# natir/br

Measured on AMD Instinct MI355X. Metric: corrected Gbases/sec at k=19, 10 kb ONT-error reads, higher is better.
Workload: dtype u64 k-mers / 1-bit set

## Files before the change

### br_amd/csrc/brx_partbuild.hip

```cpp
#include "brx_internal.hpp"
#include "brx_index.hpp"

#include <stdlib.h>
#include <string.h>
#include <atomic>

using namespace brx;

namespace {

constexpr int F_BITS = 12;
constexpr int MAX_LEVELS = 4;
constexpr int MAX_DIGIT_BITS = 9;
static_assert(MAX_DIGIT_BITS <= 9, "the digit scans of the partition passes are written for at most 512 digits");

struct Plan {
    int k, nbits, nlev;
    int bits[MAX_LEVELS];
    int rem_in[MAX_LEVELS];
    uint64_t nchild[MAX_LEVELS];
};

Plan make_plan(int k)
{
    Plan p;
    memset(&p, 0, sizeof(p));
    p.k = k;
    p.nbits = 2 * k - 1;
    const int P = p.nbits - F_BITS;
    p.nlev = (P + MAX_DIGIT_BITS - 1) / MAX_DIGIT_BITS;
    if (p.nlev < 2)
        p.nlev = 2;
    int left = P, rem = p.nbits;
    uint64_t nb = 1;
    for (int l = 0; l < p.nlev; l++) {
        int b = (left + (p.nlev - l) - 1) / (p.nlev - l);
        if (l == 0 && p.nbits - b > 32)
            b = p.nbits - 32;
        p.bits[l] = b;
        p.rem_in[l] = rem;
        rem -= b;
        left -= b;
        nb <<= b;
        p.nchild[l] = nb;
    }
    return p;
}

__device__ __forceinline__ uint32_t pack4(uint32_t w)
{
    uint32_t x = __builtin_bswap32((w >> 1) & 0x03030303u);
    x |= x >> 6;
    return (x | (x >> 12)) & 0xffu;
}

#ifndef BRX_L1_UNROLL
#define BRX_L1_UNROLL 4
#endif
#ifndef BRX_XCD_ITEMS
#define BRX_XCD_ITEMS 1
#endif
#ifndef BRX_DEBUG_BOUNDS
#define BRX_DEBUG_BOUNDS 0
#endif
#if BRX_DEBUG_BOUNDS
__device__ unsigned long long bounds_violations = 0ull;
__device__ __forceinline__ bool store_ok(uint64_t idx, uint64_t cap)
{
    if (idx >= cap) {
        atomicAdd(&bounds_violations, 1ull);
        return false;
    }
    return true;
}
#else
__device__ __forceinline__ bool store_ok(uint64_t, uint64_t) { return true; }
#endif
constexpr bool XCD_ITEMS = BRX_XCD_ITEMS != 0;
constexpr uint32_t L1_TILE = 4096;
constexpr uint32_t PACK_WORDS = L1_TILE / 16 + 4;
constexpr uint32_t BND_WORDS = (L1_TILE + 64) / 32 + 2;

__device__ __forceinline__ void pack_window(const uint8_t *__restrict__ bases, uint64_t total, uint64_t g0, uint32_t nbases,
                                            uint32_t *__restrict__ pk)
{
    const uint32_t nwords = (nbases + 15u) / 16u;
    for (uint32_t w = threadIdx.x; w < nwords; w += 256) {
        const uint64_t p = g0 + 16ull * w;
        uint32_t v[4] = {0, 0, 0, 0};
        if (p + 16 <= total) {
            uint4 q;
            __builtin_memcpy(&q, bases + p, 16);
            v[0] = q.x; v[1] = q.y; v[2] = q.z; v[3] = q.w;
        } else {
            for (uint32_t j = 0; j < 16; j++)
                if (p + j < total)
                    v[j >> 2] |= (uint32_t)bases[p + j] << (8u * (j & 3u));
        }
        pk[w] = (pack4(v[0]) << 24) | (pack4(v[1]) << 16) | (pack4(v[2]) << 8) | pack4(v[3]);
    }
}

__device__ __forceinline__ uint64_t kmer_at(const uint32_t *__restrict__ pk, uint32_t pos, int k)
{
    const uint32_t w = pos >> 4, sh = 2u * (pos & 15u);
    const uint64_t hi = ((uint64_t)pk[w] << 32) | pk[w + 1];
    const uint64_t lo = pk[w + 2];
    const uint64_t val = sh ? ((hi << sh) | (lo >> (32u - sh))) : hi;
    return val >> (64 - 2 * k);
}

struct ItemRange {
    unsigned long long first, end, step;
};
__device__ __forceinline__ ItemRange xcd_items(unsigned long long n_items)
{
    const unsigned long long G = gridDim.x, b = blockIdx.x;
    if (G < 8ull || !XCD_ITEMS)
        return {b, n_items, G};
    const unsigned long long x = b & 7ull, j = b >> 3;
    const unsigned long long R = (n_items + 7ull) >> 3;
    const unsigned long long lo = x * R;
    unsigned long long hi = lo + R;
    if (hi > n_items)
        hi = n_items;
    return {lo + j, hi, (G - x + 7ull) >> 3};
}

struct L1Args {
    const uint8_t *bases;
    const uint64_t *offsets;
    uint32_t n_reads;
    uint64_t total;
    uint32_t n_items;
    int k, nbits, bits;
    uint32_t *matrix;
    uint32_t n_ranges;
    uint64_t *rsum;
    const uint64_t *coff;
    uint32_t *keys_out;
    uint64_t out_cap;
};

__device__ __forceinline__ void l1_prepare(const L1Args &a, uint32_t item, uint32_t *pk, uint32_t *bnd, uint32_t *sh_r0,
                                           uint32_t &n_here, bool search)
{
    const uint64_t off0 = a.offsets[0];
    const uint64_t g0 = (uint64_t)item * L1_TILE;
    const uint64_t left = a.total - g0;
    n_here = (uint32_t)(left < L1_TILE ? left : L1_TILE);
    const uint32_t win = n_here + (uint32_t)a.k + 32u;
    pack_window(a.bases + off0, a.total, g0, win, pk);
    for (uint32_t w = threadIdx.x; w < BND_WORDS; w += 256)
        bnd[w] = 0;
    if (threadIdx.x == 0) {
        if (search) {
            uint32_t lo = 0, hi = a.n_reads + 1;
            while (lo < hi) {
                const uint32_t mid = lo + (hi - lo) / 2;
                if (a.offsets[mid] - off0 <= g0)
                    lo = mid + 1;
                else
                    hi = mid;
            }
            sh_r0[0] = lo;
        } else {
            sh_r0[0] += sh_r0[1];
        }
        sh_r0[1] = 0;
    }
    __syncthreads();
    const uint64_t lim = g0 + n_here + (uint64_t)a.k;
    uint32_t before_next = 0;
    for (uint32_t r = sh_r0[0] + threadIdx.x; r <= a.n_reads; r += 256) {
        const uint64_t o = a.offsets[r] - off0;
        if (o >= lim)
            break;
        const uint32_t p = (uint32_t)(o - g0);
        atomicOr(&bnd[p >> 5], 1u << (p & 31u));
        before_next += o <= g0 + L1_TILE ? 1u : 0u;
    }
    if (before_next)
        atomicAdd(&sh_r0[1], before_next);
    __syncthreads();
}

__device__ __forceinline__ void l1_range(uint32_t n_items, uint32_t &lo, uint32_t &hi)
{
    lo = (uint32_t)(((uint64_t)blockIdx.x * n_items) / gridDim.x);
    hi = (uint32_t)(((uint64_t)(blockIdx.x + 1) * n_items) / gridDim.x);
}

struct L1Next {
    uint4 q0, q1;
    uint64_t off;
    uint32_t m[(1u << MAX_DIGIT_BITS) / 256u];
};

__device__ __forceinline__ uint32_t l1_window_words(const L1Args &a, uint32_t item, uint32_t &n_here)
{
    const uint64_t left = a.total - (uint64_t)item * L1_TILE;
    n_here = (uint32_t)(left < L1_TILE ? left : L1_TILE);
    return (n_here + (uint32_t)a.k + 32u + 15u) / 16u;
}

template <bool ROW>
__device__ __forceinline__ void l1_fetch(const L1Args &a, uint64_t off0, uint32_t item, uint32_t r_first, L1Next &nx)
{
    const uint8_t *bases = a.bases + off0;
    const uint64_t g0 = (uint64_t)item * L1_TILE;
    uint32_t n_here;
    const uint32_t nwords = l1_window_words(a, item, n_here);
    const uint64_t p0 = g0 + 16ull * threadIdx.x, p1 = p0 + 16ull * 256ull;
    nx.q0 = make_uint4(0, 0, 0, 0);
    nx.q1 = make_uint4(0, 0, 0, 0);
    if (threadIdx.x < nwords && p0 + 16 <= a.total)
        __builtin_memcpy(&nx.q0, bases + p0, 16);
    if (256u + threadIdx.x < nwords && p1 + 16 <= a.total)
        __builtin_memcpy(&nx.q1, bases + p1, 16);
    const uint32_t r = r_first + threadIdx.x;
    nx.off = a.offsets[r <= a.n_reads ? r : a.n_reads];
    if (ROW) {
        const uint32_t B = 1u << a.bits;
#pragma unroll
        for (uint32_t q = 0; q < (1u << MAX_DIGIT_BITS) / 256u; q++) {
            const uint32_t b = threadIdx.x + 256u * q;
            nx.m[q] = b < B ? a.matrix[(uint64_t)item * B + b] : 0u;
        }
    }
}

template <bool ROW>
__device__ __forceinline__ void l1_landed(const L1Next &nx)
{
    asm volatile("" ::"v"(nx.q0.x), "v"(nx.q0.y), "v"(nx.q0.z), "v"(nx.q0.w), "v"(nx.q1.x), "v"(nx.q1.y), "v"(nx.q1.z), "v"(nx.q1.w),
                 "v"(nx.off));
    if (ROW) {
#pragma unroll
        for (uint32_t q = 0; q < (1u << MAX_DIGIT_BITS) / 256u; q++)
            asm volatile("" ::"v"(nx.m[q]));
    }
}

__device__ __forceinline__ uint32_t l1_pack16(const L1Args &a, uint64_t off0, const uint4 &q, uint64_t p)
{
    uint32_t v[4] = {q.x, q.y, q.z, q.w};
    if (p + 16 > a.total) {
        const uint8_t *bases = a.bases + off0;
        v[0] = v[1] = v[2] = v[3] = 0;
        for (uint32_t j = 0; j < 16; j++)
            if (p + j < a.total)
                v[j >> 2] |= (uint32_t)bases[p + j] << (8u * (j & 3u));
    }
    return (pack4(v[0]) << 24) | (pack4(v[1]) << 16) | (pack4(v[2]) << 8) | pack4(v[3]);
}

__device__ __forceinline__ void l1_consume(const L1Args &a, uint64_t off0, uint32_t item, const L1Next &nx, uint32_t r_first, uint32_t *pk,
                                           uint32_t *bnd, uint32_t *sh_r0, uint32_t &n_here)
{
    const uint64_t g0 = (uint64_t)item * L1_TILE;
    const uint32_t nwords = l1_window_words(a, item, n_here);
    if (threadIdx.x < nwords)
        pk[threadIdx.x] = l1_pack16(a, off0, nx.q0, g0 + 16ull * threadIdx.x);
    if (256u + threadIdx.x < nwords)
        pk[256u + threadIdx.x] = l1_pack16(a, off0, nx.q1, g0 + 16ull * (256u + threadIdx.x));
    for (uint32_t w = threadIdx.x; w < BND_WORDS; w += 256)
        bnd[w] = 0;
    const uint64_t lim = g0 + n_here + (uint64_t)a.k;
    const uint32_t r = r_first + threadIdx.x;
    const uint64_t o = nx.off - off0;
    const bool mine = r <= a.n_reads && o < lim;
    if (threadIdx.x == 0)
        sh_r0[1] = 0;
    if (threadIdx.x == 255)
        sh_r0[2] = mine ? 1u : 0u;
    __syncthreads();
    if (mine) {
        uint32_t p = (uint32_t)(o - g0);
        atomicOr(&bnd[p >> 5], 1u << (p & 31u));
        uint32_t before_next = o <= g0 + L1_TILE ? 1u : 0u;
        if (sh_r0[2])
            for (uint32_t r2 = r + 256u; r2 <= a.n_reads; r2 += 256u) {
                const uint64_t o2 = a.offsets[r2] - off0;
                if (o2 >= lim)
                    break;
                p = (uint32_t)(o2 - g0);
                atomicOr(&bnd[p >> 5], 1u << (p & 31u));
                before_next += o2 <= g0 + L1_TILE ? 1u : 0u;
            }
        if (before_next)
            atomicAdd(&sh_r0[1], before_next);
    }
}

__device__ __forceinline__ void l1_search(const L1Args &a, uint64_t off0, uint32_t item, uint32_t *sh_r0)
{
    if (threadIdx.x == 0) {
        const uint64_t g0 = (uint64_t)item * L1_TILE;
        uint32_t lo = 0, hi = a.n_reads + 1;
        while (lo < hi) {
            const uint32_t mid = lo + (hi - lo) / 2;
            if (a.offsets[mid] - off0 <= g0)
                lo = mid + 1;
            else
                hi = mid;
        }
        sh_r0[0] = lo;
    }
    __syncthreads();
}

__device__ __forceinline__ bool l1_valid(const uint32_t *bnd, uint32_t p, int k)
{
    const uint32_t q = p + 1u;
    const uint32_t w = q >> 5, sh = q & 31u;
    const uint64_t two = ((uint64_t)bnd[w + 1] << 32) | bnd[w];
    const uint32_t bits = (uint32_t)(two >> sh) & ((k > 1) ? ((1u << (k - 1)) - 1u) : 0u);
    return bits == 0u;
}

static_assert(L1_TILE == 256u * 16u, "l1_for_each_hash: 16 positions per thread");
template <int UNROLL = 4, typename F>
__device__ __forceinline__ void l1_for_each_hash(const uint32_t *__restrict__ pk, const uint32_t *__restrict__ bnd, uint32_t n_here,
                                                 int k, F &&f)
{
    const uint32_t p0 = threadIdx.x * 16u;
    if (p0 >= n_here)
        return;
    const uint32_t w = threadIdx.x;
    const uint64_t hi = ((uint64_t)pk[w] << 32) | pk[w + 1];
    const uint64_t lo = pk[w + 2];
    const uint64_t mask = kmask(k);
    uint64_t fwd = hi >> (64 - 2 * k);
    uint64_t rc = revcomp(fwd, k);
    uint64_t next = (hi << (2 * k)) | (2 * k >= 32 ? lo << (2 * k - 32) : lo >> (32 - 2 * k));
    const uint32_t q = p0 + 1u, wq = q >> 5, sh = q & 31u;
    uint64_t vb = ((((uint64_t)bnd[wq + 1] << 32) | bnd[wq]) >> sh) | (sh ? (uint64_t)bnd[wq + 2] << (64u - sh) : 0ull);
    const uint64_t vmask = k > 1 ? (1ull << (k - 1)) - 1ull : 0ull;
    const uint32_t left = n_here - p0 < 16u ? n_here - p0 : 16u;
    const int top = 2 * k - 2;
#pragma unroll UNROLL
    for (uint32_t j = 0; j < left; j++) {
        if ((vb & vmask) == 0ull)
            f(((popc64(fwd) & 1) ? rc : fwd) >> 1);
        const uint64_t b = next >> 62;
        next <<= 2;
        vb >>= 1;
        fwd = ((fwd << 2) | b) & mask;
        rc = (rc >> 2) | ((b ^ 2ull) << top);
    }
}

#ifndef BRX_L1HIST_WAVES
#define BRX_L1HIST_WAVES 1
#endif
constexpr uint32_t L1_OWN = ((1u << MAX_DIGIT_BITS) + 255u) / 256u;

__global__ __launch_bounds__(256, BRX_L1HIST_WAVES) void l1_hist_kernel(L1Args a)
{
    extern __shared__ uint32_t lds[];
    __shared__ uint32_t pk[PACK_WORDS];
    __shared__ uint32_t bnd[BND_WORDS];
    __shared__ uint32_t sh_r0[3];
    const uint32_t B = 1u << a.bits;
    const int shift = a.nbits - a.bits;
    uint32_t lo, hi;
    l1_range(a.n_items, lo, hi);
    uint64_t rs[L1_OWN];
#pragma unroll
    for (uint32_t q = 0; q < L1_OWN; q++)
        rs[q] = 0;
    if (lo < hi) {
        const uint64_t off0 = a.offsets[0];
        l1_search(a, off0, lo, sh_r0);
        uint32_t r_first = sh_r0[0];
        L1Next nx;
        l1_fetch<false>(a, off0, lo, r_first, nx);
        for (uint32_t b = threadIdx.x; b < B; b += 256)
            lds[b] = 0;
        uint32_t n_here;
        l1_landed<false>(nx);
        l1_consume(a, off0, lo, nx, r_first, pk, bnd, sh_r0, n_here);
        __syncthreads();
        r_first += sh_r0[1];
        l1_fetch<false>(a, off0, lo + 1 < hi ? lo + 1 : lo, r_first, nx);
        for (uint32_t item = lo; item < hi; item++) {
            l1_for_each_hash(pk, bnd, n_here, a.k, [&](uint64_t h) { atomicAdd(&lds[(uint32_t)(h >> shift)], 1u); });
            __syncthreads();
            uint32_t row[L1_OWN];
#pragma unroll
            for (uint32_t q = 0; q < L1_OWN; q++) {
                const uint32_t b = threadIdx.x + 256u * q;
                row[q] = 0;
                if (b < B) {
                    row[q] = lds[b];
                    lds[b] = 0;
                }
            }
            l1_landed<false>(nx);
            if (item + 1 < hi) {
                l1_consume(a, off0, item + 1, nx, r_first, pk, bnd, sh_r0, n_here);
                __syncthreads();
                r_first += sh_r0[1];
            }
#pragma unroll
            for (uint32_t q = 0; q < L1_OWN; q++) {
                const uint32_t b = threadIdx.x + 256u * q;
                if (b < B)
                    a.matrix[(uint64_t)item * B + b] = row[q];
                rs[q] += row[q];
            }
            l1_fetch<false>(a, off0, item + 2 < hi ? item + 2 : hi - 1, r_first, nx);
        }
    }
#pragma unroll
    for (uint32_t q = 0; q < L1_OWN; q++) {
        const uint32_t b = threadIdx.x + 256u * q;
        if (b < B && store_ok((uint64_t)blockIdx.x * B + b, (uint64_t)a.n_ranges * B))
            a.rsum[(uint64_t)blockIdx.x * B + b] = rs[q];
    }
}

__global__ __launch_bounds__(256) void col_scan_columns_kernel(uint64_t *__restrict__ part, uint32_t n_rows, uint32_t B,
                                                               uint64_t *__restrict__ coltot)
{
    __shared__ uint64_t wsum[4];
    const uint32_t b = blockIdx.x;
    const uint32_t per = (n_rows + 255u) / 256u;
    const uint32_t c0 = threadIdx.x * per;
    uint64_t mine = 0;
    for (uint32_t q = 0; q < per; q++) {
        const uint32_t c = c0 + q;
        if (c < n_rows)
            mine += part[(uint64_t)c * B + b];
    }
    uint64_t incl = mine;
    for (int d = 1; d < 64; d <<= 1) {
        const uint64_t t = __shfl_up(incl, d);
        if ((threadIdx.x & 63) >= (unsigned)d)
            incl += t;
    }
    if ((threadIdx.x & 63) == 63)
        wsum[threadIdx.x >> 6] = incl;
    __syncthreads();
    uint64_t base = 0;
    for (uint32_t w = 0; w < (threadIdx.x >> 6); w++)
        base += wsum[w];
    uint64_t run = base + incl - mine;
    for (uint32_t q = 0; q < per; q++) {
        const uint32_t c = c0 + q;
        if (c < n_rows) {
            const uint64_t v = part[(uint64_t)c * B + b];
            part[(uint64_t)c * B + b] = run;
            run += v;
        }
    }
    if (threadIdx.x == 255)
        coltot[b] = base + incl;
}

__global__ __launch_bounds__(64) void col_scan_digits_kernel(const uint64_t *__restrict__ coltot, uint32_t B, uint64_t *__restrict__ coff,
                                                             unsigned long long *__restrict__ total)
{
    uint64_t carry = 0;
    for (uint32_t b0 = 0; b0 < B; b0 += 64) {
        const uint32_t b = b0 + threadIdx.x;
        const uint64_t v = b < B ? coltot[b] : 0;
        uint64_t incl = v;
        for (int d = 1; d < 64; d <<= 1) {
            const uint64_t t = __shfl_up(incl, d);
            if (threadIdx.x >= (unsigned)d)
                incl += t;
        }
        if (b < B)
            coff[b] = carry + incl - v;
        carry += __shfl(incl, 63);
    }
    if (threadIdx.x == 0) {
        coff[B] = carry;
        *total = carry;
    }
}

template <bool TABLE>
__global__ __launch_bounds__(256) void flat_insert_kernel(L1Args a, uint32_t *__restrict__ bits, uint64_t *__restrict__ lines,
                                                          uint32_t line_shift, uint32_t m, uint32_t w,
                                                          unsigned long long *__restrict__ n_new)
{
    __shared__ uint32_t pk[PACK_WORDS];
    __shared__ uint32_t bnd[BND_WORDS];
    __shared__ uint32_t sh_r0[2];
    uint32_t added = 0;
    uint32_t lo, hi;
    l1_range(a.n_items, lo, hi);
    for (uint32_t item = lo; item < hi; item++) {
        uint32_t n_here;
        l1_prepare(a, item, pk, bnd, sh_r0, n_here, item == lo);
        for (uint32_t p = threadIdx.x; p < n_here; p += 256)
            if (l1_valid(bnd, p, a.k)) {
                const uint64_t kmer = kmer_at(pk, p, a.k);
                if (TABLE) {
                    added += table_find_or_insert(lines, line_shift, m, w, a.k, kmer) ? 1u : 0u;
                } else {
                    const uint64_t h = khash(kmer, a.k);
                    atomicOr(bits + (h >> 5), 1u << (h & 31u));
                }
            }
        __syncthreads();
    }
    if (TABLE) {
        for (int d = 32; d > 0; d >>= 1)
            added += __shfl_down(added, d);
        if ((threadIdx.x & 63) == 0 && added)
            atomicAdd(n_new, (unsigned long long)added);
    }
}

__global__ __launch_bounds__(256) void flat_count_kernel(L1Args a, uint64_t *__restrict__ lines, uint32_t *__restrict__ counts,
                                                         uint32_t line_shift, uint32_t m, uint32_t w, unsigned long long *__restrict__ n_new)
{
    __shared__ uint32_t pk[PACK_WORDS];
    __shared__ uint32_t bnd[BND_WORDS];
    __shared__ uint32_t sh_r0[2];
    uint32_t added = 0;
    uint32_t lo, hi;
    l1_range(a.n_items, lo, hi);
    for (uint32_t item = lo; item < hi; item++) {
        uint32_t n_here;
        l1_prepare(a, item, pk, bnd, sh_r0, n_here, item == lo);
        for (uint32_t p = threadIdx.x; p < n_here; p += 256)
            if (l1_valid(bnd, p, a.k)) {
                bool fresh;
                const uint64_t slot = table_find_or_claim(lines, line_shift, m, w, a.k, kmer_at(pk, p, a.k), fresh);
                added += fresh ? 1u : 0u;
                table_count_bump(counts + slot);
            }
        __syncthreads();
    }
    for (int d = 32; d > 0; d >>= 1)
        added += __shfl_down(added, d);
// ... 11 lines not shown
    seen++;
    kmer = kmer_at(pk, p, a.k);
    return table_owner_of(khash(kmer, a.k), parts) == part;
}

__global__ __launch_bounds__(256) void flat_count_slice_kernel(L1Args a, uint64_t *__restrict__ lines, uint32_t *__restrict__ counts,
                                                               uint32_t line_shift, uint32_t m, uint32_t w, uint32_t part, uint32_t parts,
                                                               unsigned long long *__restrict__ n_new,
                                                               unsigned long long *__restrict__ stats4)
{
    __shared__ uint32_t pk[PACK_WORDS];
    __shared__ uint32_t bnd[BND_WORDS];
    __shared__ uint32_t sh_r0[2];
    __shared__ uint64_t queue[4][SLICE_QUEUE];
    uint64_t *q = queue[threadIdx.x >> 6];
    const uint32_t lane = threadIdx.x & 63u;
    const unsigned long long below = (1ull << lane) - 1ull;
    uint32_t added = 0, seen = 0;
    uint32_t head = 0, queued = 0, trips = 0;
    unsigned long long walked = 0;
    uint32_t lo, hi;
    l1_range(a.n_items, lo, hi);
    for (uint32_t item = lo; item < hi; item++) {
        uint32_t n_here;
        l1_prepare(a, item, pk, bnd, sh_r0, n_here, item == lo);
        for (uint32_t p0 = 0; p0 < n_here; p0 += 256) {
            uint64_t kmer = 0;
            const bool mine = slice_take(a, pk, bnd, p0 + threadIdx.x, n_here, part, parts, kmer, seen);
            const unsigned long long mask = __ballot(mine);
            if (mine)
                q[(head + queued + (uint32_t)__popcll(mask & below)) & (SLICE_QUEUE - 1u)] = kmer;
            queued += (uint32_t)__popcll(mask);
            if (queued >= 64u) {
                __builtin_amdgcn_wave_barrier();
                const uint64_t mer = q[(head + lane) & (SLICE_QUEUE - 1u)];
                __builtin_amdgcn_wave_barrier();
                head = (head + 64u) & (SLICE_QUEUE - 1u);
                queued -= 64u;
                bool fresh;
                const uint64_t slot = table_find_or_claim(lines, line_shift, m, w, a.k, mer, fresh);
                added += fresh ? 1u : 0u;
                table_count_bump(counts + slot);
                walked += 64ull;
                trips++;
            }
        }
        __syncthreads();
    }
    if (queued) {
        __builtin_amdgcn_wave_barrier();
        if (lane < queued) {
            bool fresh;
            const uint64_t slot = table_find_or_claim(lines, line_shift, m, w, a.k, q[(head + lane) & (SLICE_QUEUE - 1u)], fresh);
            added += fresh ? 1u : 0u;
            table_count_bump(counts + slot);
        }
        walked += queued;
        trips++;
    }
    for (int d = 32; d > 0; d >>= 1) {
        added += __shfl_down(added, d);
        seen += __shfl_down(seen, d);
    }
    if (lane == 0u) {
        if (added)
            atomicAdd(n_new, (unsigned long long)added);
        if (seen)
            atomicAdd(stats4 + 0, (unsigned long long)seen);
        if (walked)
            atomicAdd(stats4 + 1, walked);
        if (trips)
            atomicAdd(stats4 + 2, (unsigned long long)trips);
        atomicAdd(stats4 + 3, 1ull);
    }
}

__global__ __launch_bounds__(256) void flat_slice_census_kernel(L1Args a, uint32_t part, uint32_t parts, unsigned long long *__restrict__ out2)
{
    __shared__ uint32_t pk[PACK_WORDS];
    __shared__ uint32_t bnd[BND_WORDS];
    __shared__ uint32_t sh_r0[2];
    uint32_t owned = 0, seen = 0;
    uint32_t lo, hi;
    l1_range(a.n_items, lo, hi);
    for (uint32_t item = lo; item < hi; item++) {
        uint32_t n_here;
        l1_prepare(a, item, pk, bnd, sh_r0, n_here, item == lo);
        for (uint32_t p = threadIdx.x; p < n_here; p += 256) {
            uint64_t kmer;
            owned += slice_take(a, pk, bnd, p, n_here, part, parts, kmer, seen) ? 1u : 0u;
        }
        __syncthreads();
    }
    for (int d = 32; d > 0; d >>= 1) {
        owned += __shfl_down(owned, d);
        seen += __shfl_down(seen, d);
    }
    if ((threadIdx.x & 63) == 0 && seen) {
        atomicAdd(out2 + 0, (unsigned long long)owned);
        atomicAdd(out2 + 1, (unsigned long long)seen);
    }
}

__device__ __forceinline__ void scan_bins_begin(uint32_t B, const uint32_t *cntv, uint32_t *sh_wsum, uint32_t &mine, uint32_t &incl)
{
    const uint32_t BPT = (B + 255u) / 256u;
    mine = 0;
    for (uint32_t q = 0; q < BPT; q++) {
        const uint32_t b = threadIdx.x * BPT + q;
        if (b < B)
            mine += cntv[b];
    }
    incl = mine;
    for (int d = 1; d < 64; d <<= 1) {
        const uint32_t t = __shfl_up(incl, d);
        if ((threadIdx.x & 63) >= (unsigned)d)
            incl += t;
    }
    if ((threadIdx.x & 63) == 63)
        sh_wsum[threadIdx.x >> 6] = incl;
}

__device__ __forceinline__ void scan_bins_end(uint32_t B, const uint32_t *cntv, uint32_t *lofs, uint32_t *lcur, const uint32_t *sh_wsum,
                                              uint32_t mine, uint32_t incl)
{
    const uint32_t BPT = (B + 255u) / 256u;
    uint32_t wbase = 0;
    for (uint32_t w = 0; w < (threadIdx.x >> 6); w++)
        wbase += sh_wsum[w];
    uint32_t run = wbase + incl - mine;
    for (uint32_t q = 0; q < BPT; q++) {
        const uint32_t b = threadIdx.x * BPT + q;
        if (b < B) {
            lofs[b] = run;
            lcur[b] = run;
            run += cntv[b];
        }
    }
}

__device__ __forceinline__ void block_scan_bins(uint32_t B, const uint32_t *cntv, uint32_t *lofs, uint32_t *lcur, uint32_t *sh_wsum)
{
    uint32_t mine, incl;
    scan_bins_begin(B, cntv, sh_wsum, mine, incl);
    __syncthreads();
    scan_bins_end(B, cntv, lofs, lcur, sh_wsum, mine, incl);
}

constexpr uint32_t L1_SECTOR = 8;

#ifndef BRX_L1SCAT_WAVES
#define BRX_L1SCAT_WAVES 5
#endif
__global__ __launch_bounds__(256, BRX_L1SCAT_WAVES) void l1_scatter_kernel(L1Args a)
{
    extern __shared__ __attribute__((aligned(16))) uint8_t lds_raw[];
    __shared__ uint32_t pk[PACK_WORDS];
    __shared__ uint32_t bnd[BND_WORDS];
    __shared__ uint32_t sh_r0[3];
    __shared__ uint32_t sh_wsum[4];
    const uint32_t T = L1_TILE;
    const uint32_t B = 1u << a.bits;
    uint32_t *stage_key = (uint32_t *)lds_raw;
    unsigned long long *gsm = (unsigned long long *)(stage_key + T);
    uint32_t *cntv = (uint32_t *)(gsm + B);
    uint32_t *lofs = cntv + B;
    uint32_t *lcur = lofs + B;
    const int shift = a.nbits - a.bits;
    const uint64_t child_mask = (1ull << shift) - 1ull;
    uint32_t lo, hi;
    l1_range(a.n_items, lo, hi);
    if (lo >= hi)
        return;
    for (uint32_t b = threadIdx.x; b < B; b += 256) {
        const unsigned long long p0 = a.coff[b] + a.rsum[(uint64_t)blockIdx.x * B + b];
        const unsigned long long ph = p0 & (L1_SECTOR - 1);
        gsm[b] = (p0 / L1_SECTOR) | (ph << 32) | (ph << 36);
    }
    uint32_t creg[L1_OWN][L1_SECTOR];
#pragma unroll
    for (uint32_t q = 0; q < L1_OWN; q++)
#pragma unroll
        for (uint32_t jj = 0; jj < L1_SECTOR; jj++)
            creg[q][jj] = 0;
    const uint64_t off0 = a.offsets[0];
    l1_search(a, off0, lo, sh_r0);
    uint32_t r_first = sh_r0[0];
    L1Next nx;
    l1_fetch<true>(a, off0, lo, r_first, nx);
    for (uint32_t item = lo; item < hi; item++) {
        l1_landed<true>(nx);
#pragma unroll
        for (uint32_t q = 0; q < L1_OWN; q++)
            if (threadIdx.x + 256u * q < B)
                cntv[threadIdx.x + 256u * q] = nx.m[q];
        uint32_t n_here;
        l1_consume(a, off0, item, nx, r_first, pk, bnd, sh_r0, n_here);
        uint32_t mine, incl;
        scan_bins_begin(B, cntv, sh_wsum, mine, incl);
        __syncthreads();
        r_first += sh_r0[1];
        scan_bins_end(B, cntv, lofs, lcur, sh_wsum, mine, incl);
        l1_fetch<true>(a, off0, item + 1 < hi ? item + 1 : item, r_first, nx);
        __syncthreads();
        l1_for_each_hash<BRX_L1_UNROLL>(pk, bnd, n_here, a.k, [&](uint64_t h) {
            const uint32_t d = (uint32_t)(h >> shift);
            const uint32_t slot = atomicAdd(&lcur[d], 1u);
            stage_key[slot] = (uint32_t)(h & child_mask);
        });
        __syncthreads();
#pragma unroll
        for (uint32_t q = 0; q < L1_OWN; q++) {
            const uint32_t d = threadIdx.x + 256u * q;
            if (d < B) {
                const unsigned long long m = gsm[d];
                const uint32_t n = cntv[d], base = lofs[d];
                const uint32_t gsx = (uint32_t)m, cc = (uint32_t)(m >> 32) & 15u, ph = (uint32_t)(m >> 36) & 15u;
                const uint32_t tot = cc + n, full = tot / L1_SECTOR, r = tot % L1_SECTOR;
                const uint32_t src = base - cc;
                uint32_t *out = a.keys_out + (unsigned long long)gsx * L1_SECTOR;
                for (uint32_t sct = 0; sct < full; sct++) {
                    uint32_t v[L1_SECTOR];
#pragma unroll
                    for (uint32_t jj = 0; jj < L1_SECTOR; jj++) {
                        const uint32_t e = L1_SECTOR * sct + jj;
                        v[jj] = e < cc ? creg[q][jj] : stage_key[src + e];
                    }
                    if (store_ok((unsigned long long)(gsx + sct) * L1_SECTOR + 7u, a.out_cap)) {
                        if (sct == 0 && ph) {
#pragma unroll
                            for (uint32_t jj = 0; jj < L1_SECTOR; jj++)
                                if (jj >= ph)
                                    out[jj] = v[jj];
                        } else {
                            uint4 *o4 = reinterpret_cast<uint4 *>(out + L1_SECTOR * sct);
                            o4[0] = make_uint4(v[0], v[1], v[2], v[3]);
                            o4[1] = make_uint4(v[4], v[5], v[6], v[7]);
                        }
                    }
                }
                if (full) {
#pragma unroll
                    for (uint32_t jj = 0; jj < L1_SECTOR; jj++)
                        creg[q][jj] = jj < r ? stage_key[src + L1_SECTOR * full + jj] : 0u;
                    gsm[d] = (unsigned long long)(gsx + full) | ((unsigned long long)r << 32);
                } else {
#pragma unroll
                    for (uint32_t jj = 0; jj < L1_SECTOR; jj++)
                        creg[q][jj] = jj < cc ? creg[q][jj] : (jj < r ? stage_key[src + jj] : 0u);
                    gsm[d] = (unsigned long long)gsx | ((unsigned long long)r << 32) | ((unsigned long long)ph << 36);
                }
            }
        }
        __syncthreads();
    }
#pragma unroll
    for (uint32_t q = 0; q < L1_OWN; q++) {
        const uint32_t d = threadIdx.x + 256u * q;
        if (d < B) {
            const unsigned long long m = gsm[d];
            const uint32_t cc = (uint32_t)(m >> 32) & 15u, ph = (uint32_t)(m >> 36) & 15u;
            const unsigned long long g = (unsigned long long)(uint32_t)m * L1_SECTOR;
#pragma unroll
            for (uint32_t jj = 0; jj < L1_SECTOR; jj++)
                if (jj >= ph && jj < cc && store_ok(g + jj, a.out_cap))
                    a.keys_out[g + jj] = creg[q][jj];
        }
    }
}

__global__ void tiles_from_offsets_kernel(const uint64_t *__restrict__ poff, uint64_t n_parents, uint32_t tile,
                                          uint32_t *__restrict__ ntiles)
{
    const uint64_t p = (uint64_t)blockIdx.x * blockDim.x + threadIdx.x;
    if (p >= n_parents)
        return;
    const uint64_t n = poff[p + 1] - poff[p];
    ntiles[p] = (uint32_t)((n + tile - 1) / tile);
}

struct LnItem {
    uint64_t lo;
    uint32_t n;
    uint32_t pad;
};

__global__ void fill_items_kernel(const uint64_t *__restrict__ poff, const uint64_t *__restrict__ item_off, uint64_t n_parents,
                                  uint32_t tile, LnItem *__restrict__ items)
{
    const uint64_t p = (uint64_t)blockIdx.x * blockDim.x + threadIdx.x;
    if (p >= n_parents)
        return;
    const uint64_t i0 = item_off[p], i1 = item_off[p + 1];
    const uint64_t k1 = poff[p + 1];
    uint64_t k = poff[p];
    for (uint64_t i = i0; i < i1; i++, k += tile) {
        LnItem it;
        it.lo = k;
        it.n = (uint32_t)(k1 - k < tile ? k1 - k : tile);
        it.pad = 0;
        items[i] = it;
    }
}

struct LnArgs {
    const uint32_t *keys_in;
    const LnItem *items;
    const unsigned long long *n_items;
    uint32_t tile;
    int rem_in, bits;
    uint32_t *matrix;
    const uint64_t *pos;
    void *keys_out;
    uint64_t in_cap, out_cap;
};

__device__ __forceinline__ uint4 ln_item_load(const LnArgs &a, unsigned long long item)
{
    return *reinterpret_cast<const uint4 *>(a.items + item);
}

__device__ __forceinline__ LnItem ln_item_get(const uint4 &v)
{
    LnItem it;
    it.lo = ((uint64_t)(uint32_t)__builtin_amdgcn_readfirstlane((int)v.y) << 32) | (uint32_t)__builtin_amdgcn_readfirstlane((int)v.x);
    it.n = (uint32_t)__builtin_amdgcn_readfirstlane((int)v.z);
    it.pad = 0;
    return it;
}

template <int KPT>
__device__ __forceinline__ void ln_load(const LnArgs &a, const LnItem &it, uint32_t (&key)[KPT])
{
#pragma unroll
    for (int q = 0; q < KPT; q++) {
        const uint32_t j = (uint32_t)q * 256u + threadIdx.x;
        const uint64_t i = it.lo + (j < it.n ? j : 0u);
        if (store_ok(i, a.in_cap))
            key[q] = a.keys_in[i];
    }
}

__device__ __forceinline__ uint32_t ln_count(const LnItem &it)
{
    return it.n > threadIdx.x ? (it.n - threadIdx.x + 255u) / 256u : 0u;
}

template <int KPT>
#ifndef BRX_LNHIST_WAVES
#define BRX_LNHIST_WAVES 1
#endif
__global__ __launch_bounds__(256, BRX_LNHIST_WAVES) void ln_hist_kernel(LnArgs a)
{
    extern __shared__ uint32_t lds[];
    const uint32_t B = 1u << a.bits;
    const int shift = a.rem_in - a.bits;
    const unsigned long long n_items = *a.n_items;
    const ItemRange ir = xcd_items(n_items);
    if (ir.first >= ir.end)
        return;
    uint4 it_raw = ln_item_load(a, ir.first);
    for (unsigned long long item = ir.first; item < ir.end; item += ir.step) {
// ... 887 lines not shown
    memset(&a, 0, sizeof(a));
    a.bases = d_bases;
    a.offsets = d_offsets;
    a.n_reads = n_reads;
    a.total = total_bases;
    a.n_items = (uint32_t)n_items64;
    a.k = k;
    return BRX_OK;
}

int flat_table_count_slice(const uint8_t *d_bases, const uint64_t *d_offsets, uint32_t n_reads, uint64_t total_bases, int k, uint64_t *table,
                           uint32_t *counts, uint32_t line_shift, uint32_t m, uint32_t part, uint32_t parts, unsigned long long *d_new,
                           unsigned long long *d_stats4, hipStream_t s)
{
    if (!total_bases || !n_reads)
        return BRX_OK;
    L1Args a;
    BRX_TRY(slice_args(d_bases, d_offsets, n_reads, total_bases, k, a));
    flat_count_slice_kernel<<<read_grid(a.n_items, 4096u), 256, 0, s>>>(a, table, counts, line_shift, m, (uint32_t)k - m + 1u, part, parts,
                                                                        d_new, d_stats4);
    BRX_HIP(hipGetLastError());
    return BRX_OK;
}

int flat_slice_census(const uint8_t *d_bases, const uint64_t *d_offsets, uint32_t n_reads, uint64_t total_bases, int k, uint32_t part,
                      uint32_t parts, unsigned long long *d_out2, hipStream_t s)
{
    if (!total_bases || !n_reads)
        return BRX_OK;
    L1Args a;
    BRX_TRY(slice_args(d_bases, d_offsets, n_reads, total_bases, k, a));
    flat_slice_census_kernel<<<read_grid(a.n_items, 4096u), 256, 0, s>>>(a, part, parts, d_out2);
    BRX_HIP(hipGetLastError());
    return BRX_OK;
}

bool part_supported(int k)
{
    return 2 * k - 1 > F_BITS && 2 * k - 1 - F_BITS <= MAX_LEVELS * MAX_DIGIT_BITS && 2 * k - 1 - MAX_DIGIT_BITS <= 32;
}

int part_begin(brx_counter *c)
{
    PartState *st = new PartState();
    c->part = st;
    st->pl = make_plan(c->k);
    const Plan &pl = st->pl;
    st->pl_wide = pl;
    if (pl.nlev == 3 && pl.bits[1] < MAX_DIGIT_BITS) {
        Plan &w = st->pl_wide;
        const int moved = MAX_DIGIT_BITS - pl.bits[1] < pl.bits[2] ? MAX_DIGIT_BITS - pl.bits[1] : pl.bits[2];
        w.bits[1] += moved;
        w.bits[2] -= moved;
        w.rem_in[2] -= moved;
        w.nchild[1] <<= moved;
    } else if (pl.nlev == 4) {
        Plan &w = st->pl_wide;
        const int P = pl.bits[0] + pl.bits[1] + pl.bits[2] + pl.bits[3];
        const int b1 = MAX_DIGIT_BITS;
        int b2 = (pl.nbits - pl.bits[0] - b1) - 20;
        if (b2 < 0)
            b2 = 0;
        const int b3 = P - pl.bits[0] - b1 - b2;
        if (b3 >= 0 && b3 <= MAX_DIGIT_BITS && b2 <= MAX_DIGIT_BITS) {
            w.bits[1] = b1;
            w.bits[2] = b2;
            w.bits[3] = b3;
            w.rem_in[2] = w.rem_in[1] - b1;
            w.rem_in[3] = w.rem_in[2] - b2;
            w.nchild[1] = w.nchild[0] << b1;
            w.nchild[2] = w.nchild[1] << b2;
            w.nchild[3] = w.nchild[2] << b3;
        }
    }
    const char *what = "partition state";
    BRX_TRY(st->d_scalars.reserve(4, 0, what));
    for (int l = 0; l < pl.nlev; l++) {
        const uint64_t nc = pl.nchild[l] > st->pl_wide.nchild[l] ? pl.nchild[l] : st->pl_wide.nchild[l];
        BRX_TRY(st->d_coff[l].reserve(nc + 1, 0, what));
    }
    BRX_TRY(st->d_l1off_all.reserve(pl.nchild[0] + 1, 0, what));
    BRX_TRY(st->d_cnts.reserve(pl.nchild[0] + 1, 0, what));
    return st->d_shift.reserve(pl.nchild[0] + 1, 0, what);
}

void part_free(brx_counter *c)
{
    delete c->part;
    c->part = nullptr;
}

int part_reset(brx_counter *c)
{
    PartState *st = c->part;
    st->view_valid = false;
    for (auto &b : st->batches)
        if (!b.borrowed())
            st->spare.push_back(std::move(b));
    st->batches.clear();
    return BRX_OK;
}

int part_l1_view(brx_counter *c, void **d_keys, void **d_l1off, uint32_t *n_buckets, uint64_t *n_keys)
{
    PartState *st = c->part;
    st->view_valid = false;
    *n_buckets = (uint32_t)st->pl.nchild[0];
    if (st->batches.empty()) {
        *d_keys = nullptr;
        *d_l1off = nullptr;
        *n_keys = 0;
        return BRX_OK;
    }
    if (st->batches.size() != 1 || st->batches[0].borrowed()) {
        set_error("l1_view needs exactly one locally counted batch (have %zu)", st->batches.size());
        return BRX_ERR_ARG;
    }
    *d_keys = st->batches[0].d_keys;
    *d_l1off = st->batches[0].d_l1off;
    *n_keys = st->batches[0].n;
    return BRX_OK;
}

int part_add_partitioned(brx_counter *c, const uint32_t *d_keys, const uint64_t *d_l1off, uint64_t n_keys)
{
    PartState *st = c->part;
    st->view_valid = false;
    if (n_keys == 0)
        return BRX_OK;
    PartBatch b;
    b.d_keys = const_cast<uint32_t *>(d_keys);
    b.d_l1off = const_cast<uint64_t *>(d_l1off);
    b.n = n_keys;
    st->batches.push_back(std::move(b));
    return BRX_OK;
}

static int ensure_matrix(PartState *st, uint64_t n_entries, uint64_t n_pos)
{
    BRX_TRY(ws_reserve(st->d_matrix, (n_entries + 1) * 4));
    BRX_TRY(ws_reserve(st->d_pos, (n_pos + 2) * 8));
    return ws_reserve(st->d_scan_tmp, scan_tmp_bytes((uint32_t)n_entries) + 64);
}

static size_t scatter_lds_bytes(uint32_t tile, int bits)
{
    const size_t B = (size_t)1 << bits;
    return (size_t)tile * 6 + B * 8 + B * 12 + 64;
}

static size_t l1_scatter_lds_bytes(int bits)
{
    const size_t B = (size_t)1 << bits;
    return (size_t)L1_TILE * 4 + B * 8 + B * 12 + 64;
}

int part_add_batch(brx_counter *c, const uint8_t *d_bases, const uint64_t *d_offsets, uint32_t n_reads,
                   uint64_t total_bases, hipStream_t s)
{
    PartState *st = c->part;
    const Plan &pl = st->pl;
    st->view_valid = false;
    if (total_bases == 0 || n_reads == 0)
        return BRX_OK;
    const uint64_t max_keys = total_bases;
    PartBatch b;
    for (size_t i = 0; i < st->spare.size(); i++)
        if (st->spare[i].cap() >= max_keys) {
            b = std::move(st->spare[i]);
            st->spare.erase(st->spare.begin() + (long)i);
            break;
        }
    if (!b.d_keys) {
        BRX_TRY(ws_reserve(b.own_keys, (max_keys + 1) * 4));
        BRX_TRY(b.own_l1off.reserve(pl.nchild[0] + 1, 0, "partition offsets"));
        b.d_keys = b.own_keys;
        b.d_l1off = b.own_l1off;
    }
    const uint32_t B = 1u << pl.bits[0];
    const uint64_t n_items64 = (total_bases + L1_TILE - 1) / L1_TILE;
    if (n_items64 * B >= (1ull << 32)) {
        set_error("batch of %llu bases is too large for one partition pass; split it", (unsigned long long)total_bases);
        return BRX_ERR_UNSUPPORTED;
    }
    const uint32_t n_items = (uint32_t)n_items64;
    const uint64_t n_entries = (uint64_t)B * n_items;
    const char *genv = getenv("BRX_L1_GRID");
    const long gev = genv ? atol(genv) : 0;
    const uint32_t want_ranges = gev > 0 ? (uint32_t)gev : 2560u;
    const uint32_t n_ranges = n_items < want_ranges ? n_items : want_ranges;
    BRX_TRY(ensure_matrix(st, n_entries, ((uint64_t)n_ranges + 1) * B));
    uint64_t *coltot = st->d_pos + (uint64_t)n_ranges * B;
    L1Args a;
    memset(&a, 0, sizeof(a));
    a.bases = d_bases;
    a.offsets = d_offsets;
    a.n_reads = n_reads;
    a.total = total_bases;
    a.n_items = n_items;
    a.k = pl.k;
    a.nbits = pl.nbits;
    a.bits = pl.bits[0];
    a.matrix = st->d_matrix;
    a.n_ranges = n_ranges;
    a.rsum = st->d_pos;
    a.coff = b.d_l1off;
    a.keys_out = b.d_keys;
    a.out_cap = b.cap();
    {
        KernelTimer t("part_l1_hist", s);
        l1_hist_kernel<<<n_ranges, 256, (size_t)B * 4, s>>>(a);
    }
    trace_stage(s, "partition level 1: histograms");
    {
        KernelTimer t("offsets_scan", s);
        col_scan_columns_kernel<<<B, 256, 0, s>>>(st->d_pos, n_ranges, B, coltot);
        col_scan_digits_kernel<<<1, 64, 0, s>>>(coltot, B, b.d_l1off, st->d_scalars + 1);
    }
    {
        KernelTimer t("part_l1_scatter", s);
        const size_t lds1 = l1_scatter_lds_bytes(a.bits);
        if (lds1 > 64 * 1024)
            BRX_HIP(hipFuncSetAttribute((const void *)l1_scatter_kernel, hipFuncAttributeMaxDynamicSharedMemorySize, (int)lds1));
        l1_scatter_kernel<<<n_ranges, 256, lds1, s>>>(a);
    }
    trace_stage(s, "partition level 1: scatter");
    BRX_HIP(hipGetLastError());
    unsigned long long tot = 0;
    BRX_HIP(hipMemcpyAsync(&tot, st->d_scalars + 1, 8, hipMemcpyDeviceToHost, s));
    BRX_HIP(hipStreamSynchronize(s));
    b.n = tot;
    st->batches.push_back(std::move(b));
    return BRX_OK;
}

template <typename OUT>
static int run_level(PartState *st, int l, const uint32_t *keys_in, const uint64_t *poff, uint64_t n_parents, uint64_t total,
                     void *keys_out, hipStream_t s, const char *tag_hist, const char *tag_scatter)
{
    const Plan &pl = st->use_wide ? st->pl_wide : st->pl;
    const uint32_t B = 1u << pl.bits[l];
    static const bool small_tiles = [] { const char *e = getenv("BRX_SMALL_TILES"); return e && *e == '1'; }();
    const uint32_t tile = (pl.bits[l] > 8 || !small_tiles) ? 8192u : 4096u;
    const uint64_t ub_items = total / tile + n_parents + 1;
    const uint64_t n_entries = (uint64_t)B * ub_items;
    if (n_entries >= (1ull << 32)) {
        set_error("partition level %d needs %llu tile counters; split the input into smaller counters", l + 1,
                  (unsigned long long)n_entries);
        return BRX_ERR_UNSUPPORTED;
    }
    {
        BRX_TRY(ws_reserve(st->d_ntiles, (n_parents + 1) * 4));
        BRX_TRY(ws_reserve(st->d_item_off, (n_parents + 2) * 8));
        BRX_TRY(ws_reserve(st->d_items, (ub_items + 1) * sizeof(LnItem)));
    }
    BRX_TRY(ensure_matrix(st, n_entries > n_parents ? n_entries : n_parents, n_entries > n_parents ? n_entries : n_parents));
    tiles_from_offsets_kernel<<<(unsigned)((n_parents + 255) / 256), 256, 0, s>>>(poff, n_parents, tile, st->d_ntiles);
    BRX_TRY(exclusive_scan_lens(st->d_ntiles, (uint32_t)n_parents, st->d_scan_tmp, st->d_item_off, st->d_scalars, s));
    fill_items_kernel<<<(unsigned)((n_parents + 255) / 256), 256, 0, s>>>(poff, st->d_item_off, n_parents, tile, st->d_items);
    trace_stage(s, tag_hist);
    BRX_HIP(hipMemsetAsync(st->d_matrix, 0, n_entries * 4, s));
    LnArgs a;
    memset(&a, 0, sizeof(a));
    a.keys_in = keys_in;
    a.in_cap = total;
    a.items = st->d_items;
    a.n_items = st->d_scalars;
    a.tile = tile;
    a.rem_in = pl.rem_in[l];
    a.bits = pl.bits[l];
    a.matrix = st->d_matrix;
    a.pos = st->d_pos;
    a.keys_out = keys_out;
    a.out_cap = total + 64;
    const int grid = 256 * 8;
    {
        KernelTimer t(tag_hist, s);
        if (tile == 8192u)
            ln_hist_kernel<32><<<grid, 256, (size_t)B * 4, s>>>(a);
        else
            ln_hist_kernel<16><<<grid, 256, (size_t)B * 4, s>>>(a);
    }
    trace_stage(s, "  histograms done");
    {
        KernelTimer t("offsets_scan", s);
        const unsigned g = n_parents < 4096 ? (unsigned)n_parents : 4096u;
        ln_colscan_kernel<<<g, 256, 0, s>>>(st->d_matrix, poff, st->d_item_off, n_parents, B, st->d_pos, st->d_coff[l]);
    }
    {
        KernelTimer t(tag_scatter, s);
        const size_t lds = scatter_lds_bytes(tile, a.bits);
        if (tile == 8192u)
            ln_scatter_kernel<32, OUT><<<grid, 256, lds, s>>>(a);
        else
            ln_scatter_kernel<16, OUT><<<grid, 256, lds, s>>>(a);
    }
    trace_stage(s, tag_scatter);
    BRX_HIP(hipGetLastError());
    return BRX_OK;
}

static int part_finish_impl(brx_counter *c, uint32_t abundance, hipStream_t s, brx_set *dst, unsigned long long *d_hist,
                            bool view = false)
{
    PartState *st = c->part;
    st->view_valid = false;
    const bool no_set = d_hist || view;
    uint64_t total = 0;
    for (auto &b : st->batches)
        total += b.n;
    const char *e_wide = getenv("BRX_WIDE_L2");
    const uint64_t wide_from = e_wide && *e_wide ? strtoull(e_wide, nullptr, 10) : 16384ull;
    const bool lazy_on = [] { const char *e = getenv("BRX_LAZY_BITS"); return !(e && *e == '0'); }();
    st->use_wide = wide_from != 0 && !no_set && dst && (dst->sparse || (index_wanted(c->k) && lazy_on)) &&
                   st->pl_wide.bits[1] != st->pl.bits[1] &&
                   (wide_from == 1 || (st->pl.nlev == 3 ? total / st->pl.nchild[1] > wide_from
                                                        : total / st->pl_wide.nchild[2] > 640));
    const Plan &pl = st->use_wide ? st->pl_wide : st->pl;
    const uint32_t B1 = (uint32_t)pl.nchild[0];

    const uint32_t *keys1 = nullptr;
    const uint64_t *l1off = nullptr;
    if (st->batches.empty() || total == 0) {
        if (view) {
            st->view_empty = true;
            st->view_valid = true;
        }
        if (no_set)
            return BRX_OK;
        if (dst->sparse) {
            BRX_TRY(dst->d_keylist_n.reserve(1, 0, "key list counter"));
            BRX_HIP(hipMemsetAsync(dst->d_keylist_n, 0, 8, s));
            keylist_mark(dst, true);
        } else {
            BRX_HIP(hipMemsetAsync(dst->d_bits, 0, dst->nwords * 4, s));
            bits_mark(dst, true);
        }
        return BRX_OK;
    } else if (st->batches.size() == 1) {
        keys1 = st->batches[0].d_keys;
        l1off = st->batches[0].d_l1off;
    } else {
        BRX_TRY(ws_reserve(st->d_merged, (total + 1) * 4));
        BRX_TRY(ensure_matrix(st, B1 + 1, B1 + 1));
        BRX_HIP(hipMemsetAsync(st->d_cnts, 0, (uint64_t)B1 * 4, s));
        for (auto &b : st->batches)
            add_counts_kernel<<<(B1 + 255) / 256, 256, 0, s>>>(b.d_l1off, B1, st->d_cnts, nullptr);
        BRX_TRY(exclusive_scan_lens(st->d_cnts, B1, st->d_scan_tmp, st->d_l1off_all, st->d_scalars + 1, s));
        BRX_HIP(hipMemsetAsync(st->d_cnts, 0, (uint64_t)B1 * 4, s));
        for (auto &b : st->batches) {
            add_counts_kernel<<<(B1 + 255) / 256, 256, 0, s>>>(b.d_l1off, B1, st->d_cnts, st->d_shift);
            merge_segments_kernel<<<B1 < 4096u ? B1 : 4096u, 256, 0, s>>>(b.d_keys, b.d_l1off, st->d_l1off_all, st->d_shift, B1,
                                                                         st->d_merged);
        }
        keys1 = st->d_merged;
        l1off = st->d_l1off_all;
    }

    BRX_TRY(ws_reserve(st->d_keys_fin, (total + 64) * 2));
    const bool emit = !no_set && (dst->sparse || index_wanted(c->k));
    const bool lazy = emit && !dst->sparse && lazy_on;
    if (emit) {
        const uint64_t div = (dst->sparse || lazy) ? abundance + 1u : (abundance + 1u > 8u ? abundance + 1u : 8u);
        const uint64_t want = total / div + (1ull << 20);
        BRX_TRY(dst->d_keylist.reserve(want, 0, "solid key list"));
        BRX_TRY(dst->d_keylist_n.reserve(1, 0, "key list counter"));
        BRX_HIP(hipMemsetAsync(dst->d_keylist_n, 0, 8, s));
    }
    static const char *hist_tag[MAX_LEVELS] = {"part_l1_hist", "part_l2_hist", "part_l3_hist", "part_l4_hist"};
    static const char *scat_tag[MAX_LEVELS] = {"part_l1_scatter", "part_l2_scatter", "part_l3_scatter", "part_l4_scatter"};
    if (pl.nlev >= 3)
        BRX_TRY(ws_reserve(st->d_keys_mid, (total + 64) * 4));
    if (pl.nlev >= 4)
        BRX_TRY(ws_reserve(st->d_keys_mid2, (total + 64) * 4));
    const uint32_t *kin = keys1;
    const uint64_t *poff = l1off;
    const bool hf_on = [] { const char *e = getenv("BRX_HASH_FINAL"); return !(e && *e == '0'); }();
// ... 166 lines not shown
```

Measured before the change: 27.57.

## Compute level-1 canonical k-mer hashes branch-free from a packed window

Replaces the serial rolling forward/revcomp loop in the level-1 histogram and scatter kernels with a per-thread window. Each of the 16 positions computes its canonical k-mer and digit directly from three packed words and their precomputed reverse complements. Parity uses prefix-XOR tricks, and validity is turned into a hold bitmask, so invalid positions go to dummy LDS bins or trash slots instead of branching. Both kernels are also templated on k and digit bits, with k=19 and k=21 specialised. This adds LDS padding and more code, and the invalid-position atomics now hit dummy bins rather than being skipped.

```diff
diff --git a/br_amd/csrc/brx_partbuild.hip b/br_amd/csrc/brx_partbuild.hip
--- a/br_amd/csrc/brx_partbuild.hip
+++ b/br_amd/csrc/brx_partbuild.hip
@@ -54,9 +54,6 @@
     return (x | (x >> 12)) & 0xffu;
 }
 
-#ifndef BRX_L1_UNROLL
-#define BRX_L1_UNROLL 4
-#endif
 #ifndef BRX_XCD_ITEMS
 #define BRX_XCD_ITEMS 1
 #endif
@@ -319,36 +316,97 @@
     return bits == 0u;
 }
 
-static_assert(L1_TILE == 256u * 16u, "l1_for_each_hash: 16 positions per thread");
-template <int UNROLL = 4, typename F>
-__device__ __forceinline__ void l1_for_each_hash(const uint32_t *__restrict__ pk, const uint32_t *__restrict__ bnd, uint32_t n_here,
-                                                 int k, F &&f)
-{
-    const uint32_t p0 = threadIdx.x * 16u;
-    if (p0 >= n_here)
-        return;
-    const uint32_t w = threadIdx.x;
-    const uint64_t hi = ((uint64_t)pk[w] << 32) | pk[w + 1];
-    const uint64_t lo = pk[w + 2];
-    const uint64_t mask = kmask(k);
-    uint64_t fwd = hi >> (64 - 2 * k);
-    uint64_t rc = revcomp(fwd, k);
-    uint64_t next = (hi << (2 * k)) | (2 * k >= 32 ? lo << (2 * k - 32) : lo >> (32 - 2 * k));
+static_assert(L1_TILE == 256u * 16u, "l1_window: 16 positions per thread");
+constexpr uint32_t L1_DUMMY = 32;
+
+struct L1Win {
+    uint32_t w[3];
+    uint32_t r[3];
+    uint32_t hold;
+    uint32_t odd;
+};
+
+__device__ __forceinline__ uint64_t win_shr(uint32_t a, uint32_t b, uint32_t c, int s)
+{
+    const uint64_t hi = ((uint64_t)a << 32) | b, lo = ((uint64_t)b << 32) | c;
+    if (s >= 96)
+        return 0ull;
+    if (s >= 32)
+        return hi >> (s - 32);
+    return s ? (lo >> s) | ((uint64_t)a << (64 - s)) : lo;
+}
+
+__device__ __forceinline__ uint32_t rc16(uint32_t x)
+{
+    const uint32_t v = __builtin_bitreverse32(x) ^ 0x55555555u;
+    return ((v >> 1) & 0x55555555u) | ((v & 0x55555555u) << 1);
+}
+
+template <int K>
+__device__ __forceinline__ L1Win l1_window(const uint32_t *__restrict__ pk, const uint32_t *__restrict__ bnd, uint32_t n_here, int k_rt)
+{
+    const int k = K ? K : k_rt;
+    const uint32_t t = threadIdx.x, p0 = t * 16u;
+    L1Win x;
+    x.w[0] = pk[t];
+    x.w[1] = pk[t + 1];
+    x.w[2] = pk[t + 2];
+    x.r[0] = rc16(x.w[2]);
+    x.r[1] = rc16(x.w[1]);
+    x.r[2] = rc16(x.w[0]);
     const uint32_t q = p0 + 1u, wq = q >> 5, sh = q & 31u;
-    uint64_t vb = ((((uint64_t)bnd[wq + 1] << 32) | bnd[wq]) >> sh) | (sh ? (uint64_t)bnd[wq + 2] << (64u - sh) : 0ull);
-    const uint64_t vmask = k > 1 ? (1ull << (k - 1)) - 1ull : 0ull;
-    const uint32_t left = n_here - p0 < 16u ? n_here - p0 : 16u;
-    const int top = 2 * k - 2;
-#pragma unroll UNROLL
-    for (uint32_t j = 0; j < left; j++) {
-        if ((vb & vmask) == 0ull)
-            f(((popc64(fwd) & 1) ? rc : fwd) >> 1);
-        const uint64_t b = next >> 62;
-        next <<= 2;
-        vb >>= 1;
-        fwd = ((fwd << 2) | b) & mask;
-        rc = (rc >> 2) | ((b ^ 2ull) << top);
-    }
+    uint64_t inv = 0ull;
+    if (k > 1) {
+        inv = ((((uint64_t)bnd[wq + 1] << 32) | bnd[wq]) >> sh) | ((uint64_t)bnd[wq + 2] << (64u - sh));
+        const int want = k - 1;
+        int have = 1;
+        for (; 2 * have <= want; have *= 2)
+            inv |= inv >> have;
+        if (have < want)
+            inv |= inv >> (want - have);
+    }
+    const uint32_t left = p0 >= n_here ? 0u : (n_here - p0 < 16u ? n_here - p0 : 16u);
+    x.hold = ~(uint32_t)inv & ((1u << left) - 1u);
+    uint32_t y[3];
+#pragma unroll
+    for (int i = 0; i < 3; i++)
+        y[i] = (x.w[i] ^ (x.w[i] >> 1)) & 0x55555555u;
+    uint32_t e = (y[0] ^ (uint32_t)win_shr(y[0], y[1], y[2], 64 - 2 * k)) >> 2;
+    e ^= e >> 2;
+    e ^= e >> 4;
+    e ^= e >> 8;
+    e ^= e >> 16;
+    const uint64_t fwd0 = win_shr(x.w[0], x.w[1], x.w[2], 96 - 2 * k) & kmask(k);
+    x.odd = e ^ (0x55555555u & (0u - (uint32_t)(popc64(fwd0) & 1)));
+    return x;
+}
+
+__device__ __forceinline__ uint32_t bit_mask(uint32_t x, int b) { return (uint32_t)((int32_t)(x << (31 - b)) >> 31); }
+__device__ __forceinline__ uint32_t mask_sel(uint32_t m, uint32_t a, uint32_t b) { return b ^ ((a ^ b) & m); }
+__device__ __forceinline__ uint64_t mask_sel(uint32_t m, uint64_t a, uint64_t b)
+{
+    return ((uint64_t)mask_sel(m, (uint32_t)(a >> 32), (uint32_t)(b >> 32)) << 32) | mask_sel(m, (uint32_t)a, (uint32_t)b);
+}
+__device__ __forceinline__ uint32_t l1_holds(const L1Win &x, int j) { return bit_mask(x.hold, j); }
+__device__ __forceinline__ uint32_t l1_odd(const L1Win &x, int j) { return bit_mask(x.odd, 30 - 2 * j); }
+
+template <bool CONST>
+__device__ __forceinline__ uint64_t l1_hash_at(const L1Win &x, int j, int k)
+{
+    const uint64_t fwd = CONST ? win_shr(x.w[0], x.w[1], x.w[2], 96 - 2 * j - 2 * k)
+                               : (win_shr(x.w[0], x.w[1], x.w[2], 34 - 2 * j) & kmask(31)) >> (62 - 2 * k);
+    const uint64_t rc = win_shr(x.r[0], x.r[1], x.r[2], 2 * j);
+    return (mask_sel(l1_odd(x, j), rc, fwd) & kmask(k)) >> 1;
+}
+
+template <bool CONST>
+__device__ __forceinline__ uint32_t l1_digit_at(const L1Win &x, int j, int k, int bits)
+{
+    const uint32_t fwd = CONST ? (uint32_t)win_shr(x.w[0], x.w[1], x.w[2], 96 - 2 * j - bits)
+                               : (uint32_t)win_shr(x.w[0], x.w[1], x.w[2], 64 - 2 * j) >> (32 - bits);
+    const uint32_t rc = CONST ? (uint32_t)win_shr(x.r[0], x.r[1], x.r[2], 2 * j + 2 * k - bits)
+                              : (uint32_t)(win_shr(x.r[0], x.r[1], x.r[2], 2 * j) >> (2 * k - bits));
+    return mask_sel(l1_odd(x, j), rc, fwd) & ((1u << bits) - 1u);
 }
 
 #ifndef BRX_L1HIST_WAVES
@@ -356,14 +414,16 @@
 #endif
 constexpr uint32_t L1_OWN = ((1u << MAX_DIGIT_BITS) + 255u) / 256u;
 
+template <int K, int BITS>
 __global__ __launch_bounds__(256, BRX_L1HIST_WAVES) void l1_hist_kernel(L1Args a)
 {
     extern __shared__ uint32_t lds[];
     __shared__ uint32_t pk[PACK_WORDS];
     __shared__ uint32_t bnd[BND_WORDS];
     __shared__ uint32_t sh_r0[3];
-    const uint32_t B = 1u << a.bits;
-    const int shift = a.nbits - a.bits;
+    const int k = K ? K : a.k, bits = K ? BITS : a.bits;
+    const uint32_t B = 1u << bits;
+    const uint32_t dummy = B + (threadIdx.x & (L1_DUMMY - 1u));
     uint32_t lo, hi;
     l1_range(a.n_items, lo, hi);
     uint64_t rs[L1_OWN];
@@ -385,7 +445,12 @@
         r_first += sh_r0[1];
         l1_fetch<false>(a, off0, lo + 1 < hi ? lo + 1 : lo, r_first, nx);
         for (uint32_t item = lo; item < hi; item++) {
-            l1_for_each_hash(pk, bnd, n_here, a.k, [&](uint64_t h) { atomicAdd(&lds[(uint32_t)(h >> shift)], 1u); });
+            {
+                const L1Win x = l1_window<K>(pk, bnd, n_here, k);
+#pragma unroll
+                for (int j = 0; j < 16; j++)
+                    atomicAdd(&lds[mask_sel(l1_holds(x, j), l1_digit_at<K != 0>(x, j, k, bits), dummy)], 1u);
+            }
             __syncthreads();
             uint32_t row[L1_OWN];
 #pragma unroll
@@ -703,6 +768,7 @@
 #ifndef BRX_L1SCAT_WAVES
 #define BRX_L1SCAT_WAVES 5
 #endif
+template <int K, int BITS>
 __global__ __launch_bounds__(256, BRX_L1SCAT_WAVES) void l1_scatter_kernel(L1Args a)
 {
     extern __shared__ __attribute__((aligned(16))) uint8_t lds_raw[];
@@ -711,14 +777,16 @@
     __shared__ uint32_t sh_r0[3];
     __shared__ uint32_t sh_wsum[4];
     const uint32_t T = L1_TILE;
-    const uint32_t B = 1u << a.bits;
+    const int k = K ? K : a.k, bits = K ? BITS : a.bits;
+    const uint32_t B = 1u << bits;
     uint32_t *stage_key = (uint32_t *)lds_raw;
-    unsigned long long *gsm = (unsigned long long *)(stage_key + T);
+    unsigned long long *gsm = (unsigned long long *)(stage_key + T + 256u);
     uint32_t *cntv = (uint32_t *)(gsm + B);
     uint32_t *lofs = cntv + B;
     uint32_t *lcur = lofs + B;
-    const int shift = a.nbits - a.bits;
+    const int shift = 2 * k - 1 - bits;
     const uint64_t child_mask = (1ull << shift) - 1ull;
+    const uint32_t dummy = B + (threadIdx.x & (L1_DUMMY - 1u)), trash = T + threadIdx.x;
     uint32_t lo, hi;
     l1_range(a.n_items, lo, hi);
     if (lo >= hi)
@@ -754,11 +822,15 @@
         scan_bins_end(B, cntv, lofs, lcur, sh_wsum, mine, incl);
         l1_fetch<true>(a, off0, item + 1 < hi ? item + 1 : item, r_first, nx);
         __syncthreads();
-        l1_for_each_hash<BRX_L1_UNROLL>(pk, bnd, n_here, a.k, [&](uint64_t h) {
-            const uint32_t d = (uint32_t)(h >> shift);
-            const uint32_t slot = atomicAdd(&lcur[d], 1u);
-            stage_key[slot] = (uint32_t)(h & child_mask);
-        });
+        {
+            const L1Win x = l1_window<K>(pk, bnd, n_here, k);
+#pragma unroll
+            for (int j = 0; j < 16; j++) {
+                const uint64_t h = l1_hash_at<K != 0>(x, j, k);
+                const uint32_t slot = atomicAdd(&lcur[mask_sel(l1_holds(x, j), (uint32_t)(h >> shift), dummy)], 1u);
+                stage_key[mask_sel(l1_holds(x, j), slot, trash)] = (uint32_t)(h & child_mask);
+            }
+        }
         __syncthreads();
 #pragma unroll
         for (uint32_t q = 0; q < L1_OWN; q++) {
@@ -1952,7 +2024,20 @@
 static size_t l1_scatter_lds_bytes(int bits)
 {
     const size_t B = (size_t)1 << bits;
-    return (size_t)L1_TILE * 4 + B * 8 + B * 12 + 64;
+    return (size_t)(L1_TILE + 256) * 4 + B * 8 + B * 12 + L1_DUMMY * 4 + 64;
+}
+
+template <int K, int BITS> static void l1_hist_launch(const L1Args &a, hipStream_t s)
+{
+    l1_hist_kernel<K, BITS><<<a.n_ranges, 256, ((size_t)(1u << a.bits) + L1_DUMMY) * 4, s>>>(a);
+}
+template <int K, int BITS> static int l1_scatter_launch(const L1Args &a, hipStream_t s)
+{
+    const size_t lds1 = l1_scatter_lds_bytes(a.bits);
+    if (lds1 > 64 * 1024)
+        BRX_HIP(hipFuncSetAttribute((const void *)l1_scatter_kernel<K, BITS>, hipFuncAttributeMaxDynamicSharedMemorySize, (int)lds1));
+    l1_scatter_kernel<K, BITS><<<a.n_ranges, 256, lds1, s>>>(a);
+    return BRX_OK;
 }
 
 int part_add_batch(brx_counter *c, const uint8_t *d_bases, const uint64_t *d_offsets, uint32_t n_reads,
@@ -2009,7 +2094,12 @@
     a.out_cap = b.cap();
     {
         KernelTimer t("part_l1_hist", s);
-        l1_hist_kernel<<<n_ranges, 256, (size_t)B * 4, s>>>(a);
+        if (a.k == 19 && a.bits == 9)
+            l1_hist_launch<19, 9>(a, s);
+        else if (a.k == 21 && a.bits == 9)
+            l1_hist_launch<21, 9>(a, s);
+        else
+            l1_hist_launch<0, 0>(a, s);
     }
     trace_stage(s, "partition level 1: histograms");
     {
@@ -2019,10 +2109,12 @@
     }
     {
         KernelTimer t("part_l1_scatter", s);
-        const size_t lds1 = l1_scatter_lds_bytes(a.bits);
-        if (lds1 > 64 * 1024)
-            BRX_HIP(hipFuncSetAttribute((const void *)l1_scatter_kernel, hipFuncAttributeMaxDynamicSharedMemorySize, (int)lds1));
-        l1_scatter_kernel<<<n_ranges, 256, lds1, s>>>(a);
+        if (a.k == 19 && a.bits == 9)
+            BRX_TRY((l1_scatter_launch<19, 9>(a, s)));
+        else if (a.k == 21 && a.bits == 9)
+            BRX_TRY((l1_scatter_launch<21, 9>(a, s)));
+        else
+            BRX_TRY((l1_scatter_launch<0, 0>(a, s)));
     }
     trace_stage(s, "partition level 1: scatter");
     BRX_HIP(hipGetLastError());
```

Result: no change. 27.81 (median of 6 runs) (+0.9%).
